# crowsonkb/k-diffusion

Hardware: AMD Instinct MI355X
Metric: images/sec, 256x256 image_transformer_v2, 50-step DPM++2M (whole job) (higher is better)
Workload: dtype f32

## Files before the change

k-diffusion_amd/csrc/attn_x3.hip:

```cpp
#include "x3_common.h"

namespace kd {
namespace x3 { extern unsigned long long* g_clk; }
namespace x3a {

using b16::bf16x8;
using b16::u32x2;
using b16::u32x4;

constexpr int DH = 64;
constexpr int NA_TH = 8, NA_TW = 16;
constexpr int ROWB = 256;
template <int KS>
struct NaGeo {
  static constexpr int HR = NA_TH + KS - 1, HC = NA_TW + KS - 1;
  static constexpr int PR = 4 + KS - 1;
  static constexpr int NKT = (PR * 16 + 31) / 32;
  static constexpr int ROWS = ((HR * HC - KS + 9 + 3) / 4) * 4;
  static constexpr int LDS = ROWS * ROWB;
  static_assert(8 + KS - 1 <= 16, "16-key patch rows");
};

struct NArgs {
  const float* qkv; float* out;
  int batch, H, W, nh;
  int warm;
  unsigned long long* clk;
};

#define KD_WAIT_VM(n) asm volatile("s_waitcnt vmcnt(" #n ")" ::: "memory")

__device__ __forceinline__ void glds16(const void* src, void* dst) {
  __builtin_amdgcn_global_load_lds((const __attribute__((address_space(1))) void*)src, (__attribute__((address_space(3))) void*)dst, 16, 0, 0);
}

__device__ __forceinline__ int rsw(int row) { return ((row & 3) << 2) | ((row >> 2) & 3); }

using s16x4 = short __attribute__((ext_vector_type(4)));
__device__ __forceinline__ u32x2 tr_read(const char* img, int addr) {
  return __builtin_bit_cast(u32x2, __builtin_amdgcn_ds_read_tr16_b64_v4i16((s16x4 __attribute__((address_space(3)))*)(img + addr)));
}
__device__ __forceinline__ float max3f(float a, float b, float c) { return __builtin_fmaxf(__builtin_fmaxf(a, b), c); }
__device__ __forceinline__ float min3f(float a, float b, float c) { return __builtin_fminf(__builtin_fminf(a, b), c); }

template <int KS>
__global__ __launch_bounds__(256, NaGeo<KS>::LDS <= 80 * 1024 ? 2 : 1) void attn_na2d_x3_kernel(const NArgs a) {
  using G = NaGeo<KS>;
  constexpr int HR = G::HR, HC = G::HC, PR = G::PR, NKT = G::NKT, ROWS = G::ROWS;
  extern __shared__ __attribute__((aligned(16))) char img[];
  const int tid = threadIdx.x, lane = tid & 63, wid = __builtin_amdgcn_readfirstlane(tid >> 6), l31 = lane & 31, h2 = lane >> 5;
  const auto warm = code_warm_begin<10240>((int)blockIdx.x < a.warm && tid < 64);
  const x3::WgStamp wgs = x3::wg_stamp_begin(a.clk);
  const int wy_ = wid >> 1, wx_ = wid & 1;
  const int tiles_x = (a.W + NA_TW - 1) / NA_TW, tiles_y = (a.H + NA_TH - 1) / NA_TH;
  int r;
  {
    const int nwg = gridDim.x, xcd = blockIdx.x & 7, k = blockIdx.x >> 3;
    const int q = nwg >> 3, rem = nwg & 7;
    r = (xcd < rem ? xcd * (q + 1) : rem * (q + 1) + (xcd - rem) * q) + k;
  }
  const int tx = r % tiles_x; r /= tiles_x;
  const int ty = r % tiles_y; r /= tiles_y;
  const int head = r % a.nh, b = r / a.nh;
  const int T = a.H * a.W;
  const size_t row_bytes = (size_t)3 * a.nh * DH * 4;
  const char* base = reinterpret_cast<const char*>(a.qkv) + (size_t)b * T * row_bytes + head * (DH * 4);
  const int ty0 = ty * NA_TH, tx0 = tx * NA_TW;
  const int hy0 = max(0, min(ty0 - KS / 2, a.H - HR)), hx0 = max(0, min(tx0 - KS / 2, a.W - HC));

  constexpr int NPC = (ROWS / 4 + 3) / 4;
  unsigned soff[NPC];
  {
    int row = 4 * wid + (lane >> 4);
    int y = row / HC, x = row % HC;
#pragma unroll
    for (int i = 0; i < NPC; ++i) {
      const int ky = min(hy0 + y, a.H - 1), kx = min(hx0 + x, a.W - 1);
      soff[i] = (unsigned)((ky * a.W + kx) * (int)row_bytes + (((lane & 15) ^ rsw(x)) << 4));
      x += 16;
      if (x >= HC) { x -= HC; ++y; }
    }
  }
  auto stage = [&](int part_bytes) {
#pragma unroll
    for (int i = 0; i < NPC; ++i) {
      const int pc = wid + 4 * i;
      if (pc < ROWS / 4) glds16(base + (size_t)soff[i] + part_bytes, img + pc * 1024);
    }
  };
  stage(a.nh * DH * 4);
  const int qy_raw = ty0 + 4 * wy_ + (l31 >> 3), qx_raw = tx0 + 8 * wx_ + (l31 & 7);
  const bool q_ok = qy_raw < a.H && qx_raw < a.W;
  const int qy = min(qy_raw, a.H - 1), qx = min(qx_raw, a.W - 1);
  const int q_tok = qy * a.W + qx;
  bf16x8 qa[4][2], ql[4];
  {
    const u32x4* qp = reinterpret_cast<const u32x4*>(base + (size_t)q_tok * row_bytes + 32 * h2);
#pragma unroll
    for (int st = 0; st < 4; ++st) {
      const u32x4 c0 = qp[4 * st], c1 = qp[4 * st + 1];
      qa[st][0] = __builtin_bit_cast(bf16x8, u32x4{c0[0], c0[1], c0[0], c0[1]});
      qa[st][1] = __builtin_bit_cast(bf16x8, u32x4{c1[0], c1[1], c1[0], c1[1]});
      ql[st] = __builtin_bit_cast(bf16x8, u32x4{c0[2], c0[3], c1[2], c1[3]});
    }
  }
  const int wy = max(0, min(qy - KS / 2, a.H - KS)) - hy0, wx = max(0, min(qx - KS / 2, a.W - KS)) - hx0;
  const int row_lo = min(max(0, min(min(ty0 + 4 * wy_, a.H - 1) - KS / 2, a.H - KS)) - hy0, HR - PR);
  const int col_lo = min(max(0, min(min(tx0 + 8 * wx_, a.W - 1) - KS / 2, a.W - KS)) - hx0, HC - (8 + KS - 1));
  const int korg = row_lo * HC + col_lo;
  float colv[8], rowv[2 * NKT];
  {
    const int r0 = wy - row_lo, c0 = wx - col_lo;
#pragma unroll
    for (int j = 0; j < 8; ++j) colv[j] = ((unsigned)((j & 3) + 8 * (j >> 2) + 4 * h2 - c0) < (unsigned)KS) ? INFINITY : -INFINITY;
#pragma unroll
    for (int p = 0; p < 2 * NKT; ++p) rowv[p] = ((unsigned)(p - r0) < (unsigned)KS) ? INFINITY : -INFINITY;
  }
  KD_WAIT_VM(0);
  code_warm_end(warm);
  KD_BARRIER();

  f32x16 S[NKT];
#pragma unroll
  for (int t = 0; t < NKT; ++t)
#pragma unroll
    for (int i = 0; i < 16; ++i) S[t][i] = 0.f;
  const int kr0 = korg + (l31 >> 4) * HC + (l31 & 15);
  const int ka0 = kr0 * ROWB + (((2 * h2) ^ rsw(col_lo + (l31 & 15))) << 4);
#pragma unroll
  for (int st = 0; st < 4; ++st) {
    bf16x8 kc0[NKT], kc1[NKT], kh[NKT];
    const char* k0p = img + (ka0 ^ (st << 6));
    const char* k1p = img + (ka0 ^ (st << 6) ^ 16);
#pragma unroll
    for (int t = 0; t < NKT; ++t) {
      const u32x4 c0 = *reinterpret_cast<const u32x4*>(k0p + t * (2 * HC * ROWB));
      const u32x4 c1 = *reinterpret_cast<const u32x4*>(k1p + t * (2 * HC * ROWB));
      kc0[t] = __builtin_bit_cast(bf16x8, c0);
      kc1[t] = __builtin_bit_cast(bf16x8, c1);
      kh[t] = __builtin_bit_cast(bf16x8, u32x4{c0[0], c0[1], c1[0], c1[1]});
    }
#pragma unroll
    for (int t = 0; t < NKT; ++t) S[t] = __builtin_amdgcn_mfma_f32_32x32x16_bf16(kc0[t], qa[st][0], S[t], 0, 0, 0);
#pragma unroll
    for (int t = 0; t < NKT; ++t) S[t] = __builtin_amdgcn_mfma_f32_32x32x16_bf16(kc1[t], qa[st][1], S[t], 0, 0, 0);
#pragma unroll
    for (int t = 0; t < NKT; ++t) S[t] = __builtin_amdgcn_mfma_f32_32x32x16_bf16(kh[t], ql[st], S[t], 0, 0, 0);
  }
  asm volatile("s_waitcnt lgkmcnt(0)" ::: "memory");
  KD_BARRIER();
  stage(2 * a.nh * DH * 4);

#pragma unroll
  for (int t = 0; t < NKT; ++t)
#pragma unroll
    for (int i = 0; i < 16; ++i) S[t][i] = min3f(S[t][i], colv[i & 7], rowv[2 * t + (i >> 3)]);
  float m = -INFINITY;
#pragma unroll
  for (int t = 0; t < NKT; ++t)
#pragma unroll
    for (int i = 0; i < 16; i += 2) m = max3f(m, S[t][i], S[t][i + 1]);
  m = fmaxf(m, __shfl_xor(m, 32, 64));
  float l;
  {
    constexpr float LOG2E = 1.4426950408889634f;
    const f32x2 mb = {-m * LOG2E, -m * LOG2E};
    f32x2 l2 = {0.f, 0.f};
#pragma unroll
    for (int t = 0; t < NKT; ++t)
#pragma unroll
      for (int i = 0; i < 16; i += 2) {
        const f32x2 x = __builtin_elementwise_fma(f32x2{S[t][i], S[t][i + 1]}, f32x2{LOG2E, LOG2E}, mb);
        const f32x2 pv = {__builtin_amdgcn_exp2f(x.x), __builtin_amdgcn_exp2f(x.y)};
        S[t][i] = pv.x;
        S[t][i + 1] = pv.y;
        l2 += pv;
      }
    l = l2.x + l2.y;
  }
  l += __shfl_xor(l, 32, 64);
  bf16x8 ph[NKT][2], pl[NKT][2];
#pragma unroll
  for (int t = 0; t < NKT; ++t)
#pragma unroll
    for (int u = 0; u < 2; ++u) {
      u32x4 hi, lo;
      x3::split8(f32x4{S[t][8 * u], S[t][8 * u + 1], S[t][8 * u + 2], S[t][8 * u + 3]},
                 f32x4{S[t][8 * u + 4], S[t][8 * u + 5], S[t][8 * u + 6], S[t][8 * u + 7]}, hi, lo);
      ph[t][u] = __builtin_bit_cast(bf16x8, hi);
      pl[t][u] = __builtin_bit_cast(bf16x8, lo);
    }
  KD_WAIT_VM(0);
  KD_BARRIER();

  f32x16 O[2];
#pragma unroll
  for (int e = 0; e < 2; ++e)
#pragma unroll
    for (int i = 0; i < 16; ++i) O[e][i] = 0.f;
  const int vr0 = korg + 4 * h2 + ((lane & 15) >> 2);
  const int vc = (lane & 3) + 4 * ((lane >> 4) & 1);
  const int va0 = vr0 * ROWB + ((vc ^ rsw(col_lo + 4 * h2 + ((lane & 15) >> 2))) << 4);
  const int vb[2][2] = {{va0, (va0 ^ 32) + 8 * ROWB}, {va0 ^ 128, ((va0 ^ 128) ^ 32) + 8 * ROWB}};
#pragma unroll
  for (int t = 0; t < NKT; ++t)
#pragma unroll
    for (int u = 0; u < 2; ++u) {
      constexpr int step = HC * ROWB;
      bf16x8 vh[2], vl[2];
#pragma unroll
      for (int e = 0; e < 2; ++e) {
        const int a0 = vb[e][0] + (2 * t + u) * step, a1 = vb[e][1] + (2 * t + u) * step;
        const u32x2 h0 = tr_read(img, a0), h1 = tr_read(img, a1), l0 = tr_read(img, a0 + 8), l1 = tr_read(img, a1 + 8);
        vh[e] = __builtin_bit_cast(bf16x8, u32x4{h0[0], h0[1], h1[0], h1[1]});
        vl[e] = __builtin_bit_cast(bf16x8, u32x4{l0[0], l0[1], l1[0], l1[1]});
      }
      O[0] = __builtin_amdgcn_mfma_f32_32x32x16_bf16(vl[0], ph[t][u], O[0], 0, 0, 0);
      O[1] = __builtin_amdgcn_mfma_f32_32x32x16_bf16(vl[1], ph[t][u], O[1], 0, 0, 0);
      O[0] = __builtin_amdgcn_mfma_f32_32x32x16_bf16(vh[0], pl[t][u], O[0], 0, 0, 0);
      O[1] = __builtin_amdgcn_mfma_f32_32x32x16_bf16(vh[1], pl[t][u], O[1], 0, 0, 0);
      O[0] = __builtin_amdgcn_mfma_f32_32x32x16_bf16(vh[0], ph[t][u], O[0], 0, 0, 0);
      O[1] = __builtin_amdgcn_mfma_f32_32x32x16_bf16(vh[1], ph[t][u], O[1], 0, 0, 0);
    }

  if (q_ok) {
    const float inv = 1.0f / l;
    float* op = a.out + ((size_t)b * T + q_tok) * (a.nh * DH) + head * DH;
#pragma unroll
    for (int e = 0; e < 2; ++e)
#pragma unroll
      for (int g = 0; g < 4; ++g)
        st16(op + e * 32 + 8 * g + 4 * h2, f32x4(f32x4{O[e][4 * g], O[e][4 * g + 1], O[e][4 * g + 2], O[e][4 * g + 3]} * inv));
  }
  x3::wg_stamp_end(wgs);
}

template <int KS>
struct NaWide {
  static constexpr int HR = NA_TH + KS - 1, HC = NA_TW + KS - 1;
  static constexpr int PR = 4 + KS - 1, PC = 20;
  static constexpr int NKT = (PR * PC + 31) / 32;
  static constexpr int ROWS = ((HR * HC + 2 * PC + 3) / 4) * 4;
  static constexpr int LDS = ROWS * ROWB;
  static_assert(8 + KS - 1 <= PC && LDS <= 160 * 1024, "patch width / LDS");
};

template <int KS>
__global__ __launch_bounds__(256, 1) void attn_na2d_x3_wide_kernel(const NArgs a) {
  using G = NaWide<KS>;
  constexpr int HR = G::HR, HC = G::HC, PR = G::PR, PC = G::PC, NKT = G::NKT, ROWS = G::ROWS;
  extern __shared__ __attribute__((aligned(16))) char img[];
  const int tid = threadIdx.x, lane = tid & 63, wid = __builtin_amdgcn_readfirstlane(tid >> 6), l31 = lane & 31, h2 = lane >> 5;
  const auto warm = code_warm_begin<16384>((int)blockIdx.x < a.warm && tid < 64);
  const int wy_ = wid >> 1, wx_ = wid & 1;
  const int tiles_x = (a.W + NA_TW - 1) / NA_TW, tiles_y = (a.H + NA_TH - 1) / NA_TH;
  int r = blockIdx.x;
  const int tx = r % tiles_x; r /= tiles_x;
  const int ty = r % tiles_y; r /= tiles_y;
  const int head = r % a.nh, b = r / a.nh;
  const int T = a.H * a.W;
  const size_t row_bytes = (size_t)3 * a.nh * DH * 4;
  const char* base = reinterpret_cast<const char*>(a.qkv) + (size_t)b * T * row_bytes + head * (DH * 4);
  const int ty0 = ty * NA_TH, tx0 = tx * NA_TW;
  const int hy0 = max(0, min(ty0 - KS / 2, a.H - HR)), hx0 = max(0, min(tx0 - KS / 2, a.W - HC));
  auto stage = [&](int part_bytes) {
    for (int pc = wid; pc < ROWS / 4; pc += 4) {
      const int row = 4 * pc + (lane >> 4);
      const int ky = min(hy0 + row / HC, a.H - 1), kx = min(hx0 + row % HC, a.W - 1);
      const char* src = base + (size_t)(unsigned)((ky * a.W + kx) * (int)row_bytes + (((lane & 15) ^ rsw(row)) << 4));
      glds16(src + part_bytes, img + pc * 1024);
    }
  };
  stage(a.nh * DH * 4);
  const int qy_raw = ty0 + 4 * wy_ + (l31 >> 3), qx_raw = tx0 + 8 * wx_ + (l31 & 7);
  const bool q_ok = qy_raw < a.H && qx_raw < a.W;
  const int qy = min(qy_raw, a.H - 1), qx = min(qx_raw, a.W - 1);
  const int q_tok = qy * a.W + qx;
  bf16x8 qh[4], ql[4];
  {
    const u32x4* qp = reinterpret_cast<const u32x4*>(base + (size_t)q_tok * row_bytes + 32 * h2);
#pragma unroll
    for (int st = 0; st < 4; ++st) {
      const u32x4 c0 = qp[4 * st], c1 = qp[4 * st + 1];
      qh[st] = __builtin_bit_cast(bf16x8, u32x4{c0[0], c0[1], c1[0], c1[1]});
      ql[st] = __builtin_bit_cast(bf16x8, u32x4{c0[2], c0[3], c1[2], c1[3]});
    }
  }
  const int wy = max(0, min(qy - KS / 2, a.H - KS)) - hy0, wx = max(0, min(qx - KS / 2, a.W - KS)) - hx0;
  const int row_lo = min(max(0, min(min(ty0 + 4 * wy_, a.H - 1) - KS / 2, a.H - KS)) - hy0, HR - PR);
  const int col_lo = min(max(0, min(min(tx0 + 8 * wx_, a.W - 1) - KS / 2, a.W - KS)) - hx0, HC - (8 + KS - 1));
  const int korg = row_lo * HC + col_lo;
  const int r0 = wy - row_lo, c0w = wx - col_lo;
  auto img_row = [&](int kl) -> int { return min(korg + (kl / PC) * HC + (kl % PC), ROWS - 1); };
  KD_WAIT_VM(0);
  code_warm_end(warm);
  KD_BARRIER();

  f32x16 S[NKT];
#pragma unroll
  for (int t = 0; t < NKT; ++t)
#pragma unroll
    for (int i = 0; i < 16; ++i) S[t][i] = 0.f;
#pragma unroll
  for (int t = 0; t < NKT; ++t) {
    const int kr = img_row(32 * t + l31);
    const int ka = kr * ROWB + (((2 * h2) ^ rsw(kr)) << 4);
#pragma unroll
    for (int st = 0; st < 4; ++st) {
      const u32x4 c0 = *reinterpret_cast<const u32x4*>(img + (ka ^ (st << 6)));
      const u32x4 c1 = *reinterpret_cast<const u32x4*>(img + (ka ^ (st << 6) ^ 16));
      const bf16x8 kh = __builtin_bit_cast(bf16x8, u32x4{c0[0], c0[1], c1[0], c1[1]});
      const bf16x8 kl = __builtin_bit_cast(bf16x8, u32x4{c0[2], c0[3], c1[2], c1[3]});
      S[t] = __builtin_amdgcn_mfma_f32_32x32x16_bf16(kl, qh[st], S[t], 0, 0, 0);
      S[t] = __builtin_amdgcn_mfma_f32_32x32x16_bf16(kh, ql[st], S[t], 0, 0, 0);
      S[t] = __builtin_amdgcn_mfma_f32_32x32x16_bf16(kh, qh[st], S[t], 0, 0, 0);
    }
  }
  asm volatile("s_waitcnt lgkmcnt(0)" ::: "memory");
  KD_BARRIER();
  stage(2 * a.nh * DH * 4);

#pragma unroll
  for (int t = 0; t < NKT; ++t)
#pragma unroll
    for (int i = 0; i < 16; ++i) {
      const int kl = 32 * t + (i & 3) + 8 * (i >> 2) + 4 * h2;
      const int pr = kl / PC, pcn = kl % PC;
      const bool valid = (unsigned)(pr - r0) < (unsigned)KS && (unsigned)(pcn - c0w) < (unsigned)KS && pr < PR;
      S[t][i] = valid ? S[t][i] : -INFINITY;
    }
  float m = -INFINITY;
#pragma unroll
  for (int t = 0; t < NKT; ++t)
#pragma unroll
    for (int i = 0; i < 16; i += 2) m = max3f(m, S[t][i], S[t][i + 1]);
  m = fmaxf(m, __shfl_xor(m, 32, 64));
  float l;
  {
    constexpr float LOG2E = 1.4426950408889634f;
    const f32x2 mb = {-m * LOG2E, -m * LOG2E};
    f32x2 l2 = {0.f, 0.f};
#pragma unroll
    for (int t = 0; t < NKT; ++t)
#pragma unroll
      for (int i = 0; i < 16; i += 2) {
        const f32x2 x = __builtin_elementwise_fma(f32x2{S[t][i], S[t][i + 1]}, f32x2{LOG2E, LOG2E}, mb);
        const f32x2 pv = {__builtin_amdgcn_exp2f(x.x), __builtin_amdgcn_exp2f(x.y)};
        S[t][i] = pv.x;
        S[t][i + 1] = pv.y;
        l2 += pv;
      }
    l = l2.x + l2.y;
  }
  l += __shfl_xor(l, 32, 64);
  KD_WAIT_VM(0);
  KD_BARRIER();

  f32x16 O[2];
#pragma unroll
  for (int e = 0; e < 2; ++e)
#pragma unroll
    for (int i = 0; i < 16; ++i) O[e][i] = 0.f;
  const int vsub = (lane & 15) >> 2;
  const int vc = (lane & 3) + 4 * ((lane >> 4) & 1);
#pragma unroll
  for (int t = 0; t < NKT; ++t)
#pragma unroll
    for (int u = 0; u < 2; ++u) {
      u32x4 phi, plo;
      x3::split8(f32x4{S[t][8 * u], S[t][8 * u + 1], S[t][8 * u + 2], S[t][8 * u + 3]},
                 f32x4{S[t][8 * u + 4], S[t][8 * u + 5], S[t][8 * u + 6], S[t][8 * u + 7]}, phi, plo);
      const bf16x8 ph = __builtin_bit_cast(bf16x8, phi), pl = __builtin_bit_cast(bf16x8, plo);
      const int k0 = 32 * t + 16 * u + 4 * h2;
      const int ra = min(img_row(k0) + vsub, ROWS - 1), rb = min(img_row(k0 + 8) + vsub, ROWS - 1);
      bf16x8 vh[2], vl[2];
#pragma unroll
      for (int e = 0; e < 2; ++e) {
        const int a0 = ra * ROWB + (((vc + 8 * e) ^ rsw(ra)) << 4), a1 = rb * ROWB + (((vc + 8 * e) ^ rsw(rb)) << 4);
        const u32x2 h0 = tr_read(img, a0), h1 = tr_read(img, a1), l0 = tr_read(img, a0 + 8), l1 = tr_read(img, a1 + 8);
        vh[e] = __builtin_bit_cast(bf16x8, u32x4{h0[0], h0[1], h1[0], h1[1]});
        vl[e] = __builtin_bit_cast(bf16x8, u32x4{l0[0], l0[1], l1[0], l1[1]});
      }
      O[0] = __builtin_amdgcn_mfma_f32_32x32x16_bf16(vl[0], ph, O[0], 0, 0, 0);
      O[1] = __builtin_amdgcn_mfma_f32_32x32x16_bf16(vl[1], ph, O[1], 0, 0, 0);
      O[0] = __builtin_amdgcn_mfma_f32_32x32x16_bf16(vh[0], pl, O[0], 0, 0, 0);
      O[1] = __builtin_amdgcn_mfma_f32_32x32x16_bf16(vh[1], pl, O[1], 0, 0, 0);
      O[0] = __builtin_amdgcn_mfma_f32_32x32x16_bf16(vh[0], ph, O[0], 0, 0, 0);
      O[1] = __builtin_amdgcn_mfma_f32_32x32x16_bf16(vh[1], ph, O[1], 0, 0, 0);
    }
  if (q_ok) {
    const float inv = 1.0f / l;
    float* op = a.out + ((size_t)b * T + q_tok) * (a.nh * DH) + head * DH;
#pragma unroll
    for (int e = 0; e < 2; ++e)
#pragma unroll
      for (int g = 0; g < 4; ++g)
        st16(op + e * 32 + 8 * g + 4 * h2, f32x4(f32x4{O[e][4 * g], O[e][4 * g + 1], O[e][4 * g + 2], O[e][4 * g + 3]} * inv));
  }
}

struct GArgs {
  const float* qkv; float* out;
  int batch, T, nh;
  int warm;
  unsigned long long* clk;
};

template <int NT>
__global__ __launch_bounds__((NT < 4 ? NT : 4) * 64, 2) void attn_global_x3_kernel(const GArgs a) {
  constexpr int QW = NT < 4 ? NT : 4, T = 32 * NT, QB = NT / QW;
  extern __shared__ __attribute__((aligned(16))) char img[];
  const int tid = threadIdx.x, lane = tid & 63, wid = __builtin_amdgcn_readfirstlane(tid >> 6), l31 = lane & 31, h2 = lane >> 5;
  const auto warm = code_warm_begin<10240>((int)blockIdx.x < a.warm && tid < 64);
  const x3::WgStamp wgs = x3::wg_stamp_begin(a.clk);
  int r;
  {
    const int nwg = gridDim.x, xcd = blockIdx.x & 7, k = blockIdx.x >> 3;
    const int q = nwg >> 3, rem = nwg & 7;
    r = (xcd < rem ? xcd * (q + 1) : rem * (q + 1) + (xcd - rem) * q) + k;
  }
  const int qb = r % QB; r /= QB;
  const int head = r % a.nh, b = r / a.nh;
  const size_t row_bytes = (size_t)3 * a.nh * DH * 4;
  const char* base = reinterpret_cast<const char*>(a.qkv) + (size_t)b * T * row_bytes + head * (DH * 4);
  auto stage = [&](int part_bytes) {
    for (int pc = wid; pc < T / 4; pc += QW) {
      const int row = 4 * pc + (lane >> 4);
      glds16(base + (size_t)row * row_bytes + part_bytes + (((lane & 15) ^ rsw(row)) << 4), img + pc * 1024);
    }
  };
  stage(a.nh * DH * 4);
  const int q_tok = 32 * (QW * qb + wid) + l31;
  bf16x8 qh[4], ql[4];
  {
    const u32x4* qp = reinterpret_cast<const u32x4*>(base + (size_t)q_tok * row_bytes + 32 * h2);
#pragma unroll
    for (int st = 0; st < 4; ++st) {
      const u32x4 c0 = qp[4 * st], c1 = qp[4 * st + 1];
      qh[st] = __builtin_bit_cast(bf16x8, u32x4{c0[0], c0[1], c1[0], c1[1]});
      ql[st] = __builtin_bit_cast(bf16x8, u32x4{c0[2], c0[3], c1[2], c1[3]});
    }
  }
  KD_WAIT_VM(0);
  code_warm_end(warm);
  KD_BARRIER();

  f32x16 S[NT];
#pragma unroll
  for (int t = 0; t < NT; ++t)
#pragma unroll
    for (int i = 0; i < 16; ++i) S[t][i] = 0.f;
  const int ka = l31 * ROWB + (((2 * h2) ^ rsw(l31)) << 4);
#pragma unroll
  for (int st = 0; st < 4; ++st) {
#pragma unroll
    for (int t0 = 0; t0 < NT; t0 += 4) {
      constexpr int TB = NT < 4 ? NT : 4;
      bf16x8 kh[TB], kl[TB];
#pragma unroll
      for (int t = 0; t < TB; ++t) {
        const char* kp = img + (t0 + t) * 32 * ROWB + (ka ^ (st << 6));
        const u32x4 c0 = *reinterpret_cast<const u32x4*>(kp);
        const u32x4 c1 = *reinterpret_cast<const u32x4*>(img + (t0 + t) * 32 * ROWB + (ka ^ (st << 6) ^ 16));
        kh[t] = __builtin_bit_cast(bf16x8, u32x4{c0[0], c0[1], c1[0], c1[1]});
        kl[t] = __builtin_bit_cast(bf16x8, u32x4{c0[2], c0[3], c1[2], c1[3]});
      }
#pragma unroll
      for (int t = 0; t < TB; ++t) S[t0 + t] = __builtin_amdgcn_mfma_f32_32x32x16_bf16(kl[t], qh[st], S[t0 + t], 0, 0, 0);
#pragma unroll
      for (int t = 0; t < TB; ++t) S[t0 + t] = __builtin_amdgcn_mfma_f32_32x32x16_bf16(kh[t], ql[st], S[t0 + t], 0, 0, 0);
#pragma unroll
      for (int t = 0; t < TB; ++t) S[t0 + t] = __builtin_amdgcn_mfma_f32_32x32x16_bf16(kh[t], qh[st], S[t0 + t], 0, 0, 0);
    }
  }
  asm volatile("s_waitcnt lgkmcnt(0)" ::: "memory");
  KD_BARRIER();
  stage(2 * a.nh * DH * 4);

  float m = -INFINITY;
#pragma unroll
  for (int t = 0; t < NT; ++t)
#pragma unroll
    for (int i = 0; i < 16; i += 2) m = max3f(m, S[t][i], S[t][i + 1]);
  m = fmaxf(m, __shfl_xor(m, 32, 64));
  float l;
  {
    constexpr float LOG2E = 1.4426950408889634f;
    const f32x2 mb = {-m * LOG2E, -m * LOG2E};
    f32x2 l2 = {0.f, 0.f};
#pragma unroll
    for (int t = 0; t < NT; ++t)
#pragma unroll
      for (int i = 0; i < 16; i += 2) {
        const f32x2 x = __builtin_elementwise_fma(f32x2{S[t][i], S[t][i + 1]}, f32x2{LOG2E, LOG2E}, mb);
        const f32x2 pv = {__builtin_amdgcn_exp2f(x.x), __builtin_amdgcn_exp2f(x.y)};
        S[t][i] = pv.x;
        S[t][i + 1] = pv.y;
        l2 += pv;
      }
    l = l2.x + l2.y;
  }
  l += __shfl_xor(l, 32, 64);
  KD_WAIT_VM(0);
  KD_BARRIER();

  f32x16 O[2];
#pragma unroll
  for (int e = 0; e < 2; ++e)
#pragma unroll
    for (int i = 0; i < 16; ++i) O[e][i] = 0.f;
  const int vr0 = 4 * h2 + ((lane & 15) >> 2);
  const int vc = (lane & 3) + 4 * ((lane >> 4) & 1);
#pragma unroll
  for (int t = 0; t < NT; ++t)
#pragma unroll
    for (int u = 0; u < 2; ++u) {
      const int vr = vr0 + 32 * t + 16 * u;
      const int va = vr * ROWB + ((vc ^ rsw(vr)) << 4);
      u32x4 phi, plo;
      x3::split8(f32x4{S[t][8 * u], S[t][8 * u + 1], S[t][8 * u + 2], S[t][8 * u + 3]},
                 f32x4{S[t][8 * u + 4], S[t][8 * u + 5], S[t][8 * u + 6], S[t][8 * u + 7]}, phi, plo);
      const bf16x8 ph = __builtin_bit_cast(bf16x8, phi), pl = __builtin_bit_cast(bf16x8, plo);
      bf16x8 vh[2], vl[2];
#pragma unroll
      for (int e = 0; e < 2; ++e) {
        const int a0 = va ^ (e << 7), a1 = (a0 ^ 32) + 8 * ROWB;
        const u32x2 h0 = tr_read(img, a0), h1 = tr_read(img, a1), l0 = tr_read(img, a0 + 8), l1 = tr_read(img, a1 + 8);
        vh[e] = __builtin_bit_cast(bf16x8, u32x4{h0[0], h0[1], h1[0], h1[1]});
        vl[e] = __builtin_bit_cast(bf16x8, u32x4{l0[0], l0[1], l1[0], l1[1]});
      }
      O[0] = __builtin_amdgcn_mfma_f32_32x32x16_bf16(vl[0], ph, O[0], 0, 0, 0);
      O[1] = __builtin_amdgcn_mfma_f32_32x32x16_bf16(vl[1], ph, O[1], 0, 0, 0);
      O[0] = __builtin_amdgcn_mfma_f32_32x32x16_bf16(vh[0], pl, O[0], 0, 0, 0);
      O[1] = __builtin_amdgcn_mfma_f32_32x32x16_bf16(vh[1], pl, O[1], 0, 0, 0);
      O[0] = __builtin_amdgcn_mfma_f32_32x32x16_bf16(vh[0], ph, O[0], 0, 0, 0);
      O[1] = __builtin_amdgcn_mfma_f32_32x32x16_bf16(vh[1], ph, O[1], 0, 0, 0);
    }
  {
    const float inv = 1.0f / l;
    float* op = a.out + ((size_t)b * T + q_tok) * (a.nh * DH) + head * DH;
#pragma unroll
    for (int e = 0; e < 2; ++e)
#pragma unroll
      for (int g = 0; g < 4; ++g)
        st16(op + e * 32 + 8 * g + 4 * h2, f32x4(f32x4{O[e][4 * g], O[e][4 * g + 1], O[e][4 * g + 2], O[e][4 * g + 3]} * inv));
  }
  x3::wg_stamp_end(wgs);
}

template <int NT>
static int launch_global(const GArgs& a, hipStream_t s) {
  constexpr int QW = NT < 4 ? NT : 4, T = 32 * NT, lds = T * ROWB;
  auto kern = attn_global_x3_kernel<NT>;
  static LdsAttr attr_set;
  attr_set.ensure(reinterpret_cast<const void*>(kern), lds);
  const long nb = (long)a.batch * a.nh * (NT / QW);
  LaunchScope prof("attn_global_x3", 4.0 * (double)a.batch * a.nh * T * T * DH, 16.0 * (double)a.batch * T * a.nh * DH, s);
  hipLaunchKernelGGL(kern, dim3((unsigned)nb), dim3(QW * 64), lds, s, a);
  return check_launch("kd_attn_global_f32(x3)");
}

}

int attn_global_x3_try(const float* qkv, float* out, int batch, int T, int nh, hipStream_t s, int* rc) {
  using namespace x3a;
  if (!option("attn_x3", 1) || (T != 64 && T != 128 && T != 256)) return 1;
  GArgs a{qkv, out, batch, T, nh, option("code_warm", KD_CODE_WARM_DEFAULT), x3::g_clk};
  *rc = T == 256 ? launch_global<8>(a, s) : (T == 128 ? launch_global<4>(a, s) : launch_global<2>(a, s));
  return 0;
}

template <int KS, bool WIDE>
static int launch_na(const x3a::NArgs& a, hipStream_t s) {
  using namespace x3a;
  constexpr int lds = WIDE ? NaWide<(WIDE ? KS : 11)>::LDS : NaGeo<(WIDE ? 7 : KS)>::LDS;
  const void* kern;
  if constexpr (WIDE) kern = reinterpret_cast<const void*>(attn_na2d_x3_wide_kernel<KS>);
  else kern = reinterpret_cast<const void*>(attn_na2d_x3_kernel<KS>);
  static LdsAttr attr_set;
  attr_set.ensure(kern, lds);
  const long nb = (long)a.batch * a.nh * ((a.H + NA_TH - 1) / NA_TH) * ((a.W + NA_TW - 1) / NA_TW);
  char nm[64] = "attn_na2d_x3";
  if (prof_on()) {
    if (KS == 7) snprintf(nm, sizeof(nm), "attn_na2d_x3 %dx%d nh=%d", a.H, a.W, a.nh);
    else snprintf(nm, sizeof(nm), "attn_na2d_x3 k%d %dx%d nh=%d", KS, a.H, a.W, a.nh);
  }
  LaunchScope prof(nm, 4.0 * a.batch * (double)a.H * a.W * a.nh * DH * KS * KS, 16.0 * a.batch * (double)a.H * a.W * a.nh * DH, s);
  if constexpr (WIDE) hipLaunchKernelGGL(attn_na2d_x3_wide_kernel<KS>, dim3((unsigned)nb), dim3(256), lds, s, a);
  else hipLaunchKernelGGL(attn_na2d_x3_kernel<KS>, dim3((unsigned)nb), dim3(256), lds, s, a);
  return check_launch("kd_attn_na2d_f32(x3)");
}

int attn_na2d_x3_try(const float* qkv, float* out, int batch, int H, int W, int nh, int ks, hipStream_t s, int* rc) {
  using namespace x3a;
  if (!option("attn_x3", 1)) return 1;
  NArgs a{qkv, out, batch, H, W, nh, option("code_warm", KD_CODE_WARM_DEFAULT), x3::g_clk};
  switch (ks) {
    case 3: *rc = launch_na<3, false>(a, s); return 0;
    case 5: *rc = launch_na<5, false>(a, s); return 0;
    case 7: *rc = launch_na<7, false>(a, s); return 0;
    case 9: *rc = launch_na<9, false>(a, s); return 0;
    case 11: *rc = launch_na<11, true>(a, s); return 0;
    case 13: *rc = launch_na<13, true>(a, s); return 0;
    default: return 1;
  }
}

}

KD_TEXT_PAD(attn_x3)
```

Measured before the change: 229.5.

## Stage K/V halves in half-width LDS rows to fit three workgroups per CU

The neighborhood-attention kernel now stages K and V in two 128-byte halves of the head dimension instead of full 256-byte rows. This halves LDS per workgroup so three workgroups fit per CU, and launch bounds move to 3 to match. The cost is extra barriers and extra staging rounds. The change also adds a new swizzle for the narrower rows, recomputes offsets when registers are tight, splits the V accumulation and store per half, and makes the stamp pointer wave-uniform.

```diff
diff --git a/k-diffusion_amd/csrc/attn_x3.hip b/k-diffusion_amd/csrc/attn_x3.hip
--- a/k-diffusion_amd/csrc/attn_x3.hip
+++ b/k-diffusion_amd/csrc/attn_x3.hip
@@ -11,14 +11,17 @@
 constexpr int DH = 64;
 constexpr int NA_TH = 8, NA_TW = 16;
 constexpr int ROWB = 256;
+constexpr int HROWB = 128;
 template <int KS>
 struct NaGeo {
   static constexpr int HR = NA_TH + KS - 1, HC = NA_TW + KS - 1;
   static constexpr int PR = 4 + KS - 1;
   static constexpr int NKT = (PR * 16 + 31) / 32;
-  static constexpr int ROWS = ((HR * HC - KS + 9 + 3) / 4) * 4;
-  static constexpr int LDS = ROWS * ROWB;
+  static constexpr int ROWS = ((HR * HC - KS + 9 + 7) / 8) * 8;
+  static constexpr int LDS = ROWS * HROWB;
   static_assert(8 + KS - 1 <= 16, "16-key patch rows");
+  static_assert(HC % 2 == 0 && HC >= 16, "hsw: even halo width (image row parity = column parity), 32 rows per staging round");
+  static_assert(3 * LDS <= 160 * 1024, "three workgroups per CU");
 };
 
 struct NArgs {
@@ -36,6 +39,8 @@
 
 __device__ __forceinline__ int rsw(int row) { return ((row & 3) << 2) | ((row >> 2) & 3); }
 
+__device__ __forceinline__ int hsw(int x) { return (((x >> 1) & 1) << 2) | ((x >> 2) & 3); }
+
 using s16x4 = short __attribute__((ext_vector_type(4)));
 __device__ __forceinline__ u32x2 tr_read(const char* img, int addr) {
   return __builtin_bit_cast(u32x2, __builtin_amdgcn_ds_read_tr16_b64_v4i16((s16x4 __attribute__((address_space(3)))*)(img + addr)));
@@ -44,13 +49,18 @@
 __device__ __forceinline__ float min3f(float a, float b, float c) { return __builtin_fminf(__builtin_fminf(a, b), c); }
 
 template <int KS>
-__global__ __launch_bounds__(256, NaGeo<KS>::LDS <= 80 * 1024 ? 2 : 1) void attn_na2d_x3_kernel(const NArgs a) {
+__global__ __launch_bounds__(256, 3) void attn_na2d_x3_kernel(const NArgs a) {
   using G = NaGeo<KS>;
   constexpr int HR = G::HR, HC = G::HC, PR = G::PR, NKT = G::NKT, ROWS = G::ROWS;
   extern __shared__ __attribute__((aligned(16))) char img[];
   const int tid = threadIdx.x, lane = tid & 63, wid = __builtin_amdgcn_readfirstlane(tid >> 6), l31 = lane & 31, h2 = lane >> 5;
   const auto warm = code_warm_begin<10240>((int)blockIdx.x < a.warm && tid < 64);
-  const x3::WgStamp wgs = x3::wg_stamp_begin(a.clk);
+  x3::WgStamp wgs = x3::wg_stamp_begin(a.clk);
+  {
+    const unsigned long long sp = reinterpret_cast<unsigned long long>(wgs.slot);
+    wgs.slot = reinterpret_cast<unsigned long long*>(((unsigned long long)__builtin_amdgcn_readfirstlane((unsigned)(sp >> 32)) << 32) |
+                                                     (unsigned)__builtin_amdgcn_readfirstlane((unsigned)sp));
+  }
   const int wy_ = wid >> 1, wx_ = wid & 1;
   const int tiles_x = (a.W + NA_TW - 1) / NA_TW, tiles_y = (a.H + NA_TH - 1) / NA_TH;
   int r;
@@ -68,54 +78,57 @@
   const int ty0 = ty * NA_TH, tx0 = tx * NA_TW;
   const int hy0 = max(0, min(ty0 - KS / 2, a.H - HR)), hx0 = max(0, min(tx0 - KS / 2, a.W - HC));
 
-  constexpr int NPC = (ROWS / 4 + 3) / 4;
-  unsigned soff[NPC];
-  {
-    int row = 4 * wid + (lane >> 4);
+  constexpr int NPC = (ROWS / 8 + 3) / 4;
+  constexpr bool HOLD = NPC <= 10;
+  auto src_offsets = [&](unsigned (&off)[NPC]) {
+    int ln = lane;
+    if constexpr (!HOLD) asm volatile("" : "+v"(ln));
+    int row = 8 * wid + (ln >> 3);
     int y = row / HC, x = row % HC;
 #pragma unroll
     for (int i = 0; i < NPC; ++i) {
       const int ky = min(hy0 + y, a.H - 1), kx = min(hx0 + x, a.W - 1);
-      soff[i] = (unsigned)((ky * a.W + kx) * (int)row_bytes + (((lane & 15) ^ rsw(x)) << 4));
-      x += 16;
+      off[i] = (unsigned)((ky * a.W + kx) * (int)row_bytes + (((ln & 7) ^ hsw(x)) << 4));
+      x += 32;
       if (x >= HC) { x -= HC; ++y; }
-    }
-  }
+      if (x >= HC) { x -= HC; ++y; }
+    }
+  };
+  unsigned soff[NPC];
+  if constexpr (HOLD) src_offsets(soff);
   auto stage = [&](int part_bytes) {
+    const unsigned long long pa = reinterpret_cast<unsigned long long>(base) + (unsigned)part_bytes;
+    const char* pb = reinterpret_cast<const char*>(((unsigned long long)__builtin_amdgcn_readfirstlane((unsigned)(pa >> 32)) << 32) |
+                                                   (unsigned)__builtin_amdgcn_readfirstlane((unsigned)pa));
+    if constexpr (!HOLD) src_offsets(soff);
 #pragma unroll
     for (int i = 0; i < NPC; ++i) {
       const int pc = wid + 4 * i;
-      if (pc < ROWS / 4) glds16(base + (size_t)soff[i] + part_bytes, img + pc * 1024);
-    }
-  };
-  stage(a.nh * DH * 4);
+      if (pc < ROWS / 8) glds16(pb + soff[i], img + pc * 1024);
+    }
+  };
   const int qy_raw = ty0 + 4 * wy_ + (l31 >> 3), qx_raw = tx0 + 8 * wx_ + (l31 & 7);
   const bool q_ok = qy_raw < a.H && qx_raw < a.W;
   const int qy = min(qy_raw, a.H - 1), qx = min(qx_raw, a.W - 1);
   const int q_tok = qy * a.W + qx;
-  bf16x8 qa[4][2], ql[4];
-  {
-    const u32x4* qp = reinterpret_cast<const u32x4*>(base + (size_t)q_tok * row_bytes + 32 * h2);
-#pragma unroll
-    for (int st = 0; st < 4; ++st) {
-      const u32x4 c0 = qp[4 * st], c1 = qp[4 * st + 1];
-      qa[st][0] = __builtin_bit_cast(bf16x8, u32x4{c0[0], c0[1], c0[0], c0[1]});
-      qa[st][1] = __builtin_bit_cast(bf16x8, u32x4{c1[0], c1[1], c1[0], c1[1]});
-      ql[st] = __builtin_bit_cast(bf16x8, u32x4{c0[2], c0[3], c1[2], c1[3]});
-    }
-  }
+  bf16x8 qa[2][2], ql[2];
+  auto load_q = [&](int half) {
+    const u32x4* qp = reinterpret_cast<const u32x4*>(base + (size_t)q_tok * row_bytes + 32 * h2 + 128 * half);
+#pragma unroll
+    for (int s = 0; s < 2; ++s) {
+      const u32x4 c0 = qp[4 * s], c1 = qp[4 * s + 1];
+      qa[s][0] = __builtin_bit_cast(bf16x8, u32x4{c0[0], c0[1], c0[0], c0[1]});
+      qa[s][1] = __builtin_bit_cast(bf16x8, u32x4{c1[0], c1[1], c1[0], c1[1]});
+      ql[s] = __builtin_bit_cast(bf16x8, u32x4{c0[2], c0[3], c1[2], c1[3]});
+    }
+  };
+  const int kpart = a.nh * DH * 4, vpart = 2 * a.nh * DH * 4;
+  stage(kpart);
+  load_q(0);
   const int wy = max(0, min(qy - KS / 2, a.H - KS)) - hy0, wx = max(0, min(qx - KS / 2, a.W - KS)) - hx0;
   const int row_lo = min(max(0, min(min(ty0 + 4 * wy_, a.H - 1) - KS / 2, a.H - KS)) - hy0, HR - PR);
   const int col_lo = min(max(0, min(min(tx0 + 8 * wx_, a.W - 1) - KS / 2, a.W - KS)) - hx0, HC - (8 + KS - 1));
   const int korg = row_lo * HC + col_lo;
-  float colv[8], rowv[2 * NKT];
-  {
-    const int r0 = wy - row_lo, c0 = wx - col_lo;
-#pragma unroll
-    for (int j = 0; j < 8; ++j) colv[j] = ((unsigned)((j & 3) + 8 * (j >> 2) + 4 * h2 - c0) < (unsigned)KS) ? INFINITY : -INFINITY;
-#pragma unroll
-    for (int p = 0; p < 2 * NKT; ++p) rowv[p] = ((unsigned)(p - r0) < (unsigned)KS) ? INFINITY : -INFINITY;
-  }
   KD_WAIT_VM(0);
   code_warm_end(warm);
   KD_BARRIER();
@@ -126,35 +139,51 @@
 #pragma unroll
     for (int i = 0; i < 16; ++i) S[t][i] = 0.f;
   const int kr0 = korg + (l31 >> 4) * HC + (l31 & 15);
-  const int ka0 = kr0 * ROWB + (((2 * h2) ^ rsw(col_lo + (l31 & 15))) << 4);
-#pragma unroll
-  for (int st = 0; st < 4; ++st) {
-    bf16x8 kc0[NKT], kc1[NKT], kh[NKT];
-    const char* k0p = img + (ka0 ^ (st << 6));
-    const char* k1p = img + (ka0 ^ (st << 6) ^ 16);
-#pragma unroll
-    for (int t = 0; t < NKT; ++t) {
-      const u32x4 c0 = *reinterpret_cast<const u32x4*>(k0p + t * (2 * HC * ROWB));
-      const u32x4 c1 = *reinterpret_cast<const u32x4*>(k1p + t * (2 * HC * ROWB));
-      kc0[t] = __builtin_bit_cast(bf16x8, c0);
-      kc1[t] = __builtin_bit_cast(bf16x8, c1);
-      kh[t] = __builtin_bit_cast(bf16x8, u32x4{c0[0], c0[1], c1[0], c1[1]});
-    }
-#pragma unroll
-    for (int t = 0; t < NKT; ++t) S[t] = __builtin_amdgcn_mfma_f32_32x32x16_bf16(kc0[t], qa[st][0], S[t], 0, 0, 0);
-#pragma unroll
-    for (int t = 0; t < NKT; ++t) S[t] = __builtin_amdgcn_mfma_f32_32x32x16_bf16(kc1[t], qa[st][1], S[t], 0, 0, 0);
-#pragma unroll
-    for (int t = 0; t < NKT; ++t) S[t] = __builtin_amdgcn_mfma_f32_32x32x16_bf16(kh[t], ql[st], S[t], 0, 0, 0);
-  }
-  asm volatile("s_waitcnt lgkmcnt(0)" ::: "memory");
-  KD_BARRIER();
-  stage(2 * a.nh * DH * 4);
-
-#pragma unroll
-  for (int t = 0; t < NKT; ++t)
-#pragma unroll
-    for (int i = 0; i < 16; ++i) S[t][i] = min3f(S[t][i], colv[i & 7], rowv[2 * t + (i >> 3)]);
+  const int ka0 = kr0 * HROWB + (((2 * h2) ^ hsw(col_lo + (l31 & 15))) << 4);
+  auto k_phase = [&]() {
+#pragma unroll
+    for (int s = 0; s < 2; ++s) {
+      bf16x8 kc0[NKT], kc1[NKT], kh[NKT];
+      const char* k0p = img + (ka0 ^ (s << 6));
+      const char* k1p = img + (ka0 ^ (s << 6) ^ 16);
+#pragma unroll
+      for (int t = 0; t < NKT; ++t) {
+        const u32x4 c0 = *reinterpret_cast<const u32x4*>(k0p + t * (2 * HC * HROWB));
+        const u32x4 c1 = *reinterpret_cast<const u32x4*>(k1p + t * (2 * HC * HROWB));
+        kc0[t] = __builtin_bit_cast(bf16x8, c0);
+        kc1[t] = __builtin_bit_cast(bf16x8, c1);
+        kh[t] = __builtin_bit_cast(bf16x8, u32x4{c0[0], c0[1], c1[0], c1[1]});
+      }
+#pragma unroll
+      for (int t = 0; t < NKT; ++t) S[t] = __builtin_amdgcn_mfma_f32_32x32x16_bf16(kc0[t], qa[s][0], S[t], 0, 0, 0);
+#pragma unroll
+      for (int t = 0; t < NKT; ++t) S[t] = __builtin_amdgcn_mfma_f32_32x32x16_bf16(kc1[t], qa[s][1], S[t], 0, 0, 0);
+#pragma unroll
+      for (int t = 0; t < NKT; ++t) S[t] = __builtin_amdgcn_mfma_f32_32x32x16_bf16(kh[t], ql[s], S[t], 0, 0, 0);
+    }
+    asm volatile("s_waitcnt lgkmcnt(0)" ::: "memory");
+    KD_BARRIER();
+  };
+  k_phase();
+  stage(kpart + 128);
+  load_q(1);
+  KD_WAIT_VM(0);
+  KD_BARRIER();
+  k_phase();
+  stage(vpart);
+
+  {
+    float colv[8], rowv[2 * NKT];
+    const int r0 = wy - row_lo, c0 = wx - col_lo;
+#pragma unroll
+    for (int j = 0; j < 8; ++j) colv[j] = ((unsigned)((j & 3) + 8 * (j >> 2) + 4 * h2 - c0) < (unsigned)KS) ? INFINITY : -INFINITY;
+#pragma unroll
+    for (int p = 0; p < 2 * NKT; ++p) rowv[p] = ((unsigned)(p - r0) < (unsigned)KS) ? INFINITY : -INFINITY;
+#pragma unroll
+    for (int t = 0; t < NKT; ++t)
+#pragma unroll
+      for (int i = 0; i < 16; ++i) S[t][i] = min3f(S[t][i], colv[i & 7], rowv[2 * t + (i >> 3)]);
+  }
   float m = -INFINITY;
 #pragma unroll
   for (int t = 0; t < NKT; ++t)
@@ -200,39 +229,43 @@
     for (int i = 0; i < 16; ++i) O[e][i] = 0.f;
   const int vr0 = korg + 4 * h2 + ((lane & 15) >> 2);
   const int vc = (lane & 3) + 4 * ((lane >> 4) & 1);
-  const int va0 = vr0 * ROWB + ((vc ^ rsw(col_lo + 4 * h2 + ((lane & 15) >> 2))) << 4);
-  const int vb[2][2] = {{va0, (va0 ^ 32) + 8 * ROWB}, {va0 ^ 128, ((va0 ^ 128) ^ 32) + 8 * ROWB}};
-#pragma unroll
-  for (int t = 0; t < NKT; ++t)
-#pragma unroll
-    for (int u = 0; u < 2; ++u) {
-      constexpr int step = HC * ROWB;
-      bf16x8 vh[2], vl[2];
-#pragma unroll
-      for (int e = 0; e < 2; ++e) {
-        const int a0 = vb[e][0] + (2 * t + u) * step, a1 = vb[e][1] + (2 * t + u) * step;
+  const int va0 = vr0 * HROWB + ((vc ^ hsw(col_lo + 4 * h2 + ((lane & 15) >> 2))) << 4);
+  const int vb[2] = {va0, (va0 ^ 32) + 8 * HROWB};
+  auto v_phase = [&](f32x16& o) {
+#pragma unroll
+    for (int t = 0; t < NKT; ++t)
+#pragma unroll
+      for (int u = 0; u < 2; ++u) {
+        constexpr int step = HC * HROWB;
+        const int a0 = vb[0] + (2 * t + u) * step, a1 = vb[1] + (2 * t + u) * step;
         const u32x2 h0 = tr_read(img, a0), h1 = tr_read(img, a1), l0 = tr_read(img, a0 + 8), l1 = tr_read(img, a1 + 8);
-        vh[e] = __builtin_bit_cast(bf16x8, u32x4{h0[0], h0[1], h1[0], h1[1]});
-        vl[e] = __builtin_bit_cast(bf16x8, u32x4{l0[0], l0[1], l1[0], l1[1]});
-      }
-      O[0] = __builtin_amdgcn_mfma_f32_32x32x16_bf16(vl[0], ph[t][u], O[0], 0, 0, 0);
-      O[1] = __builtin_amdgcn_mfma_f32_32x32x16_bf16(vl[1], ph[t][u], O[1], 0, 0, 0);
-      O[0] = __builtin_amdgcn_mfma_f32_32x32x16_bf16(vh[0], pl[t][u], O[0], 0, 0, 0);
-      O[1] = __builtin_amdgcn_mfma_f32_32x32x16_bf16(vh[1], pl[t][u], O[1], 0, 0, 0);
-      O[0] = __builtin_amdgcn_mfma_f32_32x32x16_bf16(vh[0], ph[t][u], O[0], 0, 0, 0);
-      O[1] = __builtin_amdgcn_mfma_f32_32x32x16_bf16(vh[1], ph[t][u], O[1], 0, 0, 0);
-    }
-
-  if (q_ok) {
-    const float inv = 1.0f / l;
-    float* op = a.out + ((size_t)b * T + q_tok) * (a.nh * DH) + head * DH;
-#pragma unroll
-    for (int e = 0; e < 2; ++e)
-#pragma unroll
-      for (int g = 0; g < 4; ++g)
-        st16(op + e * 32 + 8 * g + 4 * h2, f32x4(f32x4{O[e][4 * g], O[e][4 * g + 1], O[e][4 * g + 2], O[e][4 * g + 3]} * inv));
-  }
-  x3::wg_stamp_end(wgs);
+        const bf16x8 vh = __builtin_bit_cast(bf16x8, u32x4{h0[0], h0[1], h1[0], h1[1]});
+        const bf16x8 vl = __builtin_bit_cast(bf16x8, u32x4{l0[0], l0[1], l1[0], l1[1]});
+        o = __builtin_amdgcn_mfma_f32_32x32x16_bf16(vl, ph[t][u], o, 0, 0, 0);
+        o = __builtin_amdgcn_mfma_f32_32x32x16_bf16(vh, pl[t][u], o, 0, 0, 0);
+        o = __builtin_amdgcn_mfma_f32_32x32x16_bf16(vh, ph[t][u], o, 0, 0, 0);
+      }
+  };
+  const float inv = 1.0f / l;
+  auto store = [&](int e, const f32x16& o) {
+    int qt = q_tok;
+    asm volatile("" : "+v"(qt));
+    float* op = a.out + ((size_t)b * T + qt) * (a.nh * DH) + head * DH;
+    if (q_ok) {
+#pragma unroll
+      for (int g = 0; g < 4; ++g) st16(op + e * 32 + 8 * g + 4 * h2, f32x4(f32x4{o[4 * g], o[4 * g + 1], o[4 * g + 2], o[4 * g + 3]} * inv));
+    }
+  };
+  v_phase(O[0]);
+  asm volatile("s_waitcnt lgkmcnt(0)" ::: "memory");
+  KD_BARRIER();
+  stage(vpart + 128);
+  store(0, O[0]);
+  KD_WAIT_VM(0);
+  KD_BARRIER();
+  v_phase(O[1]);
+  store(1, O[1]);
+  if (tid == 0) x3::wg_stamp_end(wgs);
 }
 
 template <int KS>
```

After: 230.6, median of 6. Within noise of the previous version (+0.5%).
